# sota-zk-labs/zkp-implementation

Measured on AMD Instinct MI355X. Metric: G1 MSM scalar-muls/sec, higher is better.
Workload: dtype u32 (unsaturated 28-bit-limb Montgomery, 381-bit Fq; 64-bit accumulate)

## Files before the change

zkp-implementation_amd/csrc/msm.hpp:

```cpp
#pragma once
#include "g1.hpp"
#include "g1_28.hpp"
#include "fq28_inv.hpp"
#include "msm_plan.hpp"
#include "glv.hpp"

namespace zkp {

#define ZKP_AT(f, o) offsetof(MsmGeom, f) == o
static_assert(sizeof(MsmGeom) == 160 && ZKP_AT(c, 0) && ZKP_AT(nwin, 4) && ZKP_AT(nb, 8) && ZKP_AT(nchunk, 12) && ZKP_AT(n, 16) && ZKP_AT(chunk, 24) &&
              ZKP_AT(ns, 32) && ZKP_AT(plane_stride, 40) && ZKP_AT(nslice, 48) && ZKP_AT(shared, 52) && ZKP_AT(run_limit, 56) && ZKP_AT(piece, 60) &&
              ZKP_AT(resume, 64) && ZKP_AT(off, 68) && ZKP_AT(interleave, 140) && ZKP_AT(split_log, 144) && ZKP_AT(more, 148) && ZKP_AT(glv, 152), "MsmGeom layout");
#undef ZKP_AT
static_assert(sizeof(SortGeom) == 8 && offsetof(SortGeom, lo_bits) == 0 && offsetof(SortGeom, nhi) == 4, "SortGeom layout");

ZKP_DEV uint64_t bucket_cap(const MsmGeom& g) { return (uint64_t)g.nwin * g.nb; }

#ifdef ZKP_MSM_CHECK
__device__ uint32_t g_msm_check[32];
ZKP_DEV bool msm_check_fail(int cls, uint32_t v0, uint32_t v1) {
    if (atomicAdd(&g_msm_check[cls * 4], 1u) == 0) { g_msm_check[cls * 4 + 1] = v0; g_msm_check[cls * 4 + 2] = v1; }
    return true;
}
#endif
struct DigitSources {
    const Fr* scalars[MSM_MAX_BATCH];
};
ZKP_DEV void msm_recode(const uint32_t (&k)[8], bool skip, const MsmGeom& g, uint32_t nwin1, uint32_t group, uint64_t i,
                        uint32_t* __restrict__ digits) {
    const uint32_t win_off = group * nwin1;
    uint32_t carry = 0;
    for (uint32_t w = 0; w < nwin1; w++) {
        const uint32_t lo = g.off[w], width = (uint32_t)g.off[w + 1] - lo;
        const uint32_t limb = lo >> 5, sh = lo & 31;
        uint64_t v = 0;
#pragma unroll
        for (int q = 0; q < 8; q++) {
            if (q == (int)limb) v |= (uint64_t)k[q];
            if (q == (int)limb + 1) v |= (uint64_t)k[q] << 32;
        }
        uint32_t u = ((uint32_t)(v >> sh) & ((1u << width) - 1)) + carry;
        uint32_t enc;
        if (u > (1u << (width - 1))) {
            enc = (((1u << width) - u) << 1) | 1u;
            carry = 1;
        } else {
            enc = u << 1;
            carry = 0;
        }
        digits[(uint64_t)(win_off + w) * g.ns + i] = skip ? 0u : enc;
    }
}
__global__ __launch_bounds__(MSM_THREADS) void msm_digits_kernel(DigitSources src, const uint8_t* __restrict__ base_inf, MsmGeom g,
                                                                uint32_t nwin1, uint32_t* __restrict__ digits) {
    const uint64_t i = (uint64_t)blockIdx.x * MSM_THREADS + threadIdx.x;
    if (i >= g.ns) return;
    Fr k = from_mont(src.scalars[blockIdx.y][i]);
    const bool skip = base_inf != nullptr && base_inf[i] != 0;
    msm_recode(k.l, skip, g, nwin1, blockIdx.y, i, digits);
}
__global__ __launch_bounds__(MSM_THREADS) void msm_digits_glv_kernel(DigitSources src, const uint8_t* __restrict__ base_inf, MsmGeom g,
                                                                    uint32_t nwin1, uint32_t* __restrict__ digits) {
    const uint64_t i = (uint64_t)blockIdx.x * MSM_THREADS + threadIdx.x;
    if (i >= g.ns) return;
    const Fr k = from_mont(src.scalars[blockIdx.y][i]);
    const bool skip = base_inf != nullptr && base_inf[i] != 0;
    const GlvHalves h = glv_split(k.l);
    const uint32_t k1[8] = {h.k1[0], h.k1[1], h.k1[2], h.k1[3], 0, 0, 0, 0}, k2[8] = {h.k2[0], h.k2[1], h.k2[2], h.k2[3], 0, 0, 0, 0};
    msm_recode(k1, skip, g, nwin1, 2 * blockIdx.y, i, digits);
    msm_recode(k2, skip, g, nwin1, 2 * blockIdx.y + 1, i, digits);
}


ZKP_DEV void wave_exclusive_scan(const uint32_t* cnt, uint32_t* base, uint32_t nbins, uint32_t lane) {
    const uint32_t per = (nbins + 63) / 64;
    const uint32_t b0 = lane * per < nbins ? lane * per : nbins;
    const uint32_t b1 = b0 + per < nbins ? b0 + per : nbins;
    uint32_t sum = 0;
    for (uint32_t k = b0; k < b1; k++) sum += cnt[k];
    uint32_t inc = sum;
#pragma unroll
    for (int off = 1; off < 64; off <<= 1) {
        const uint32_t t = __shfl_up(inc, off);
        if (lane >= (uint32_t)off) inc += t;
    }
    uint32_t run = inc - sum;
    for (uint32_t k = b0; k < b1; k++) {
        const uint32_t v = cnt[k];
        base[k] = run;
        run += v;
    }
    if (lane == 63) base[nbins] = run;
}

__global__ __launch_bounds__(1024) void msm_parthist_kernel(const uint32_t* __restrict__ digits, MsmGeom g, SortGeom sg,
                                                            uint32_t* __restrict__ cntA) {
    __shared__ uint32_t h[SORT_MAX_PART];
    const uint32_t q = blockIdx.x, w = blockIdx.y;
    for (uint32_t k = threadIdx.x; k < sg.nhi; k += blockDim.x) h[k] = 0;
    __syncthreads();
    const uint64_t begin = (uint64_t)q * g.chunk;
    const uint64_t end = begin + g.chunk < g.n ? begin + g.chunk : g.n;
    const uint32_t* d = digits + (uint64_t)w * g.n;
    const uint64_t nt = blockDim.x;
    for (uint64_t i = begin + threadIdx.x; i < end; i += 4 * nt) {
        uint32_t e[4];
#pragma unroll
        for (int k = 0; k < 4; k++) e[k] = i + k * nt < end ? d[i + k * nt] : 0u;
#pragma unroll
        for (int k = 0; k < 4; k++) {
            const uint32_t b = e[k] >> 1;
            if (b) atomicAdd(&h[(b - 1) >> sg.lo_bits], 1u);
        }
    }
    __syncthreads();
    uint32_t* out = cntA + ((uint64_t)w * g.nchunk + q) * sg.nhi;
    for (uint32_t k = threadIdx.x; k < sg.nhi; k += blockDim.x) out[k] = h[k];
}

__global__ __launch_bounds__(1024) void msm_partprefix_kernel(uint32_t* __restrict__ cntA, MsmGeom g, SortGeom sg,
                                                              uint32_t* __restrict__ tot) {
    __shared__ uint32_t part[16][64];
    const uint32_t w = blockIdx.y, h = threadIdx.x & 63, qg = threadIdx.x >> 6;
    const uint32_t hi = blockIdx.x * 64 + h;
    const bool live = hi < sg.nhi;
    uint32_t* cw = cntA + (uint64_t)w * g.nchunk * sg.nhi;
    const uint32_t per = (g.nchunk + 15) / 16;
    const uint32_t q0 = qg * per < g.nchunk ? qg * per : g.nchunk;
    const uint32_t q1 = q0 + per < g.nchunk ? q0 + per : g.nchunk;
    uint32_t sum = 0;
    if (live)
        for (uint32_t q = q0; q < q1; q++) sum += cw[(uint64_t)q * sg.nhi + hi];
    part[qg][h] = sum;
    __syncthreads();
    uint32_t run = 0, total = 0;
    for (uint32_t k = 0; k < 16; k++) {
        if (k < qg) run += part[k][h];
        total += part[k][h];
    }
    if (live) {
        for (uint32_t q = q0; q < q1; q++) {
            uint32_t* p = cw + (uint64_t)q * sg.nhi + hi;
            const uint32_t v = *p;
            *p = run;
            run += v;
        }
        if (qg == 0) tot[(uint64_t)w * sg.nhi + hi] = total;
    }
}

__global__ __launch_bounds__(64) void msm_partstart_kernel(const uint32_t* __restrict__ tot, SortGeom sg,
                                                           uint32_t* __restrict__ pstart, uint32_t* __restrict__ ghist,
                                                           uint32_t* __restrict__ tail_barrier) {
    __shared__ uint32_t t[SORT_MAX_PART + 1];
    uint32_t* base = t;
    const uint32_t w = blockIdx.x;
    for (uint32_t k = threadIdx.x; k < 256; k += 64) {
        ghist[w * 256 + k] = 0;
        ghist[(gridDim.x + w) * 256 + k] = 0;
    }
    if (threadIdx.x == 0) tail_barrier[w * PYR_BAR_STRIDE] = 0;
    for (uint32_t k = threadIdx.x; k < sg.nhi; k += 64) t[k] = tot[(uint64_t)w * sg.nhi + k];
    __syncthreads();
    wave_exclusive_scan(t, base, sg.nhi, threadIdx.x);
    __syncthreads();
    for (uint32_t k = threadIdx.x; k <= sg.nhi; k += 64) pstart[(uint64_t)w * (sg.nhi + 1) + k] = base[k];
}

#ifndef ZKP_BS_TILE
#define ZKP_BS_TILE 16384
#endif
constexpr int BS_TILE = ZKP_BS_TILE;
constexpr int BS_PER = BS_TILE / 1024;
constexpr int SORT_MAX_BINS = 1024;

template <int PS_TILE>
__global__ __launch_bounds__(1024) void msm_partscatter_kernel(const uint32_t* __restrict__ digits, MsmGeom g, SortGeom sg,
                                                               const uint32_t* __restrict__ cntA,
                                                               const uint32_t* __restrict__ pstart,
                                                               uint2* __restrict__ entries) {
    constexpr int PS_PER = PS_TILE / 1024;
    extern __shared__ uint4 zkp_smem[];
    uint2* stage = reinterpret_cast<uint2*>(zkp_smem);
    uint16_t* part = reinterpret_cast<uint16_t*>(stage + PS_TILE);
    uint32_t* cur = reinterpret_cast<uint32_t*>(part + PS_TILE);
    uint32_t* cnt = cur + sg.nhi;
    uint32_t* base = cnt + sg.nhi;
    const uint32_t q = blockIdx.x, w = blockIdx.y, tid = threadIdx.x;
    for (uint32_t k = tid; k < sg.nhi; k += 1024)
        cur[k] = pstart[(uint64_t)w * (sg.nhi + 1) + k] + cntA[((uint64_t)w * g.nchunk + q) * sg.nhi + k];
    const uint64_t begin = (uint64_t)q * g.chunk;
    const uint64_t end = begin + g.chunk < g.n ? begin + g.chunk : g.n;
    const uint32_t* d = digits + (uint64_t)w * g.n;
    uint2* out = entries + (uint64_t)w * g.n;
    const uint32_t lo_mask = (1u << sg.lo_bits) - 1;
    for (uint64_t t0 = begin; t0 < end; t0 += PS_TILE) {
        for (uint32_t k = tid; k < sg.nhi; k += 1024) cnt[k] = 0;
        __syncthreads();
        uint32_t e[PS_PER], rk[PS_PER];
#pragma unroll
        for (int k = 0; k < PS_PER; k++) {
            const uint64_t i = t0 + tid + (uint64_t)k * 1024;
            e[k] = i < end ? d[i] : 0u;
        }
#pragma unroll
        for (int k = 0; k < PS_PER; k++) {
            const uint32_t b = e[k] >> 1;
            rk[k] = b ? atomicAdd(&cnt[(b - 1) >> sg.lo_bits], 1u) : 0u;
        }
        __syncthreads();
        if (tid < 64) wave_exclusive_scan(cnt, base, sg.nhi, tid);
        __syncthreads();
#pragma unroll
        for (int k = 0; k < PS_PER; k++) {
            const uint32_t b = e[k] >> 1;
            if (b) {
                const uint32_t p = (b - 1) >> sg.lo_bits;
                const uint32_t pos = base[p] + rk[k];
                stage[pos] = make_uint2((uint32_t)(t0 - 0 + tid + (uint64_t)k * 1024) | ((e[k] & 1u) << 31), (b - 1) & lo_mask);
// ... 39 lines not shown
        for (int k = 0; k < 4; k++)
            if (y[k] != 0xffffffffu) atomicAdd(&cnt[y[k]], 1u);
    }
    __syncthreads();
    if (tid < lo_n) atomicAdd(&szh[255 - (cnt[tid] < 255 ? cnt[tid] : 255)], 1u);
    if (tid < 64) wave_exclusive_scan(cnt, h, lo_n, tid);
    __syncthreads();
    if (tid < 256 && szh[tid]) atomicAdd(&ghist[w * 256 + tid], szh[tid]);
    if (tid < lo_n) h[tid] += begin;
    __syncthreads();
    uint32_t* sw = start + (uint64_t)w * (g.nb + 2);
    if (tid < lo_n) sw[(hi << sg.lo_bits) + tid + 1] = h[tid];
    if (hi == 0 && tid == 0) sw[0] = 0;
    if (hi == sg.nhi - 1 && tid == 0) sw[g.nb + 1] = end;
    __syncthreads();
    uint32_t* out = sorted + (uint64_t)w * g.n;
    for (uint32_t t0 = begin; t0 < end; t0 += BS_TILE) {
        if (tid < lo_n) cnt[tid] = 0;
        __syncthreads();
        uint2 e[BS_PER];
        uint32_t rk[BS_PER];
#pragma unroll
        for (int k = 0; k < BS_PER; k++) {
            const uint32_t i = t0 + tid + k * 1024;
            e[k] = i < end ? in[i] : make_uint2(0u, 0xffffffffu);
        }
#pragma unroll
        for (int k = 0; k < BS_PER; k++) rk[k] = e[k].y != 0xffffffffu ? atomicAdd(&cnt[e[k].y], 1u) : 0u;
        __syncthreads();
        if (tid < 64) wave_exclusive_scan(cnt, base, lo_n, tid);
        __syncthreads();
#pragma unroll
        for (int k = 0; k < BS_PER; k++)
            if (e[k].y != 0xffffffffu) {
                const uint32_t pos = base[e[k].y] + rk[k];
                stage[pos] = e[k].x;
                bin[pos] = (uint16_t)e[k].y;
            }
        __syncthreads();
        const uint32_t total = base[lo_n];
        for (uint32_t j = tid; j < total; j += 1024) {
            const uint32_t p = bin[j];
#ifdef ZKP_MSM_CHECK
            if ((uint64_t)h[p] + (j - base[p]) >= g.n && msm_check_fail(1, h[p] + (j - base[p]), p)) continue;
#endif
            out[h[p] + (j - base[p])] = stage[j];
        }
        __syncthreads();
        if (tid < lo_n) h[tid] += cnt[tid];
    }
}


__global__ __launch_bounds__(1024) void msm_rank_kernel(const uint32_t* __restrict__ start, MsmGeom g,
                                                        const uint32_t* __restrict__ ghist, uint32_t* __restrict__ gcur,
                                                        uint32_t* __restrict__ perm) {
    __shared__ uint32_t hist[256], base[256], gh[256], first[257];
    const uint32_t w = blockIdx.y, tid = threadIdx.x;
    const uint32_t* sw = start + (uint64_t)w * (g.nb + 2);
    if (tid < 256) {
        hist[tid] = 0;
        gh[tid] = ghist[w * 256 + tid];
    }
    __syncthreads();
    if (tid < 64) wave_exclusive_scan(gh, first, 256, tid);
    const uint32_t b = 1 + blockIdx.x * 1024 + tid;
    uint32_t bin = 0, rk = 0;
    if (b <= g.nb) {
        const uint32_t sz = sw[b + 1] - sw[b];
        bin = 255 - (sz < 255 ? sz : 255);
        rk = atomicAdd(&hist[bin], 1u);
    }
    __syncthreads();
    if (tid < 256 && hist[tid]) base[tid] = first[tid] + atomicAdd(&gcur[w * 256 + tid], hist[tid]);
    __syncthreads();
#ifdef ZKP_MSM_CHECK
    if (b <= g.nb && base[bin] + rk >= g.nb && msm_check_fail(5, base[bin] + rk, b)) return;
#endif
    if (b <= g.nb) perm[(uint64_t)w * g.nb + base[bin] + rk] = b;
}

__global__ __launch_bounds__(1024) void msm_order_kernel(const uint32_t* __restrict__ start, MsmGeom g,
                                                         const uint32_t* __restrict__ ghist,
                                                         const uint32_t* __restrict__ perm, uint32_t* __restrict__ over,
                                                         uint32_t* __restrict__ over_b, uint32_t* __restrict__ over_off,
                                                         uint4* __restrict__ desc, uint32_t over_cap, uint32_t desc_cap) {
    __shared__ uint32_t s_over[2], gh[256], first[257];
    const uint32_t w = blockIdx.x, tid = threadIdx.x, nt = blockDim.x;
    const uint32_t* sw = start + (uint64_t)w * (g.nb + 2);
    const uint32_t* pw = perm + (uint64_t)w * g.nb;
    if (tid < 256) gh[tid] = ghist[w * 256 + tid];
    __syncthreads();
    if (tid < 64) wave_exclusive_scan(gh, first, 256, tid);
    __syncthreads();
    if (tid == 0) {
        const uint32_t limit_bin = g.run_limit < 254 ? g.run_limit : 254;
        s_over[0] = first[255 - limit_bin];
    }
    __syncthreads();
    const uint32_t n_over = s_over[0] < over_cap ? s_over[0] : over_cap;
#ifdef ZKP_MSM_CHECK
    if (tid == 0 && s_over[0] > g.nb) msm_check_fail(7, s_over[0], over_cap);
#endif
    uint32_t* ob = over_b + (uint64_t)w * over_cap;
    uint32_t* oo = over_off + (uint64_t)w * (over_cap + 1);
    {
        __shared__ uint32_t part[1024];
        const uint32_t per = (n_over + nt - 1) / nt;
        const uint32_t r0 = tid * per < n_over ? tid * per : n_over;
        const uint32_t r1 = r0 + per < n_over ? r0 + per : n_over;
        uint32_t local = 0;
        for (uint32_t r = r0; r < r1; r++) {
            const uint32_t b = pw[r];
#ifdef ZKP_MSM_CHECK
            if ((b == 0 || b > g.nb) && msm_check_fail(6, b, r)) continue;
#endif
            const uint32_t sz = sw[b + 1] - sw[b];
            local += sz > g.run_limit ? (sz + g.piece - 1) / g.piece : 0;
        }
        part[tid] = local;
        __syncthreads();
        for (uint32_t off = 1; off < nt; off <<= 1) {
            const uint32_t v = tid >= off ? part[tid - off] : 0;
            __syncthreads();
            part[tid] += v;
            __syncthreads();
        }
        uint32_t run = tid ? part[tid - 1] : 0;
        for (uint32_t r = r0; r < r1; r++) {
            const uint32_t b = pw[r];
#ifdef ZKP_MSM_CHECK
            if (b == 0 || b > g.nb) { ob[r] = 1; oo[r] = run; continue; }
#endif
            const uint32_t sz = sw[b + 1] - sw[b];
            ob[r] = b;
            oo[r] = run;
            run += sz > g.run_limit ? (sz + g.piece - 1) / g.piece : 0;
        }
        if (tid == nt - 1) {
            const uint32_t total = part[nt - 1];
            oo[n_over] = total;
            s_over[1] = total;
            over[2 * w] = n_over;
            over[2 * w + 1] = total < desc_cap ? total : desc_cap;
        }
    }
    __syncthreads();
    const uint32_t n_pieces = s_over[1] < desc_cap ? s_over[1] : desc_cap;
    uint4* dw = desc + (uint64_t)w * desc_cap;
    for (uint32_t j = tid; j < n_pieces; j += nt) {
        uint32_t lo = 0, hi = n_over;
        while (hi - lo > 1) {
            const uint32_t mid = (lo + hi) >> 1;
            if (oo[mid] <= j) lo = mid; else hi = mid;
        }
        const uint32_t b = ob[lo], p = j - oo[lo];
        const uint32_t first = sw[b] + p * g.piece;
        const uint32_t last = first + g.piece < sw[b + 1] ? first + g.piece : sw[b + 1];
        dw[j] = make_uint4(b, p, first, last);
    }
}

__global__ __launch_bounds__(MSM_THREADS) void g1_to_internal_kernel(const uint4* __restrict__ in, uint64_t n,
                                                                    uint4* __restrict__ out) {
    const uint64_t i = (uint64_t)blockIdx.x * MSM_THREADS + threadIdx.x;
    if (i >= n) return;
    G1Affine p = G1Affine::load(in + i * 6);
#pragma unroll 1
    for (int k = 0; k < 8; k++) {
        p.x = dbl(p.x);
        p.y = dbl(p.y);
    }
    A28 q;
    q.x = fq28_from_sat(p.x);
    q.y = fq28_from_sat(p.y);
    q.store(out + i * 8);
}

struct SliceOffsets {
    uint16_t off[36];
};
__global__ __launch_bounds__(MSM_THREADS) void g1_expand_planes_kernel(uint4* __restrict__ planes, uint4* __restrict__ scratch,
                                                                      uint64_t off, uint64_t cnt, uint64_t plane_stride,
                                                                      uint32_t nplanes, SliceOffsets so) {
    const uint64_t j = (uint64_t)blockIdx.x * MSM_THREADS + threadIdx.x;
    if (j >= cnt) return;
    const uint64_t i = off + j;
    auto slot = [&](uint32_t s, uint32_t t) { return scratch + (((uint64_t)s * 3 + t) * cnt + j) * 4; };
    const A28 p0 = A28::load(planes + i * 8);
    X28 x = g1_28_double_affine(p0);
    Fq28 run = Fq28::one();
#pragma unroll 1
    for (uint32_t s = 1; s < nplanes; s++) {
#pragma unroll 1
        for (uint32_t k = (s == 1 ? 1u : 0u), c = (uint32_t)so.off[s] - so.off[s - 1]; k < c; k++) x = g1_28_double(x);
        A28 raw;
        raw.x = x.x;
        raw.y = x.y;
        raw.store(planes + (s * plane_stride + i) * 8);
        run.store(slot(s, 2));
        x.zz.store(slot(s, 0));
        x.zzz.store(slot(s, 1));
        run = run * x.zzz;
    }
    Fq28 inv = fq28_inverse_gcd(run);
#pragma unroll 1
    for (uint32_t s = nplanes - 1; s >= 1; s--) {
        const Fq28 zi3 = inv * Fq28::load(slot(s, 2));
        inv = inv * Fq28::load(slot(s, 1));
        const Fq28 zi = zi3 * Fq28::load(slot(s, 0));
        const Fq28 zi2 = zi * zi;
        uint4* dst = planes + (s * plane_stride + i) * 8;
        const A28 raw = A28::load(dst);
// ... 491 lines not shown
```

zkp-implementation_amd/csrc/msm_host.inc:

```

#ifdef ZKP_MSM_CHECK
#define MSM_TRACE(stream, ridx, what) do { hipError_t e_ = hipStreamSynchronize(stream); fprintf(stderr, "ZKP_MSM_CHECK range %llu: %s done (%d)\n", (unsigned long long)(ridx), what, (int)e_); } while (0)
#else
#define MSM_TRACE(stream, ridx, what) do { } while (0)
#endif

struct MsmFeed {
    const uint64_t* h_scalars;
    hipStream_t copy_stream;
    hipEvent_t ev;
    MsmFeedRanges ranges;
};

struct RangeBuffers {
    uint32_t *sorted, *start, *perm;
    uint4* desc;
    uint32_t *over, *over_b, *over_off;
};

struct MsmPass {
    const MsmPlan& p;
    const zkp_bases* bases;
    const Fr* const* scalars;
    size_t count;
// ... 65 lines not shown
                      });
        }
        hipError_t e1 = hipMemcpyAsync(dst, feed->h_scalars, 32 * p.lens[0], hipMemcpyHostToDevice, feed->copy_stream);
        if (e1 == hipSuccess) e1 = hipEventRecord(feed->ev, feed->copy_stream);
        up.release(e1 == hipSuccess);
        HIPCHK(e1);
        return ZKP_OK;
    }

    int walk() {
        if (p.overlap) {
            ZCHK(cx.sort_stream.ensure(hipStreamNonBlocking));
            for (Event* e : {&cx.ev_sort[0], &cx.ev_sort[1], &cx.ev_acc[0], &cx.ev_acc[1], &cx.ev_begin}) ZCHK(e->ensure(hipEventDisableTiming));
            sst = cx.sort_stream;
            HIPCHK(hipEventRecord(cx.ev_begin, st));
            HIPCHK(hipStreamWaitEvent(sst, cx.ev_begin, 0));
        }
        for (size_t ridx = 0; ridx < p.lens.size(); ridx++) {
            const MsmRange r = range_geom(p, ridx);
            const size_t par = r.set;
            const RangeBuffers rb = range_buffers(par);
            if (p.overlap && ridx >= 2) HIPCHK(hipStreamWaitEvent(sst, cx.ev_acc[par], 0));
            if (feed) {
                if (ridx == 0)
                    ZCHK(feed_first_range());
                else if (!up.wait_issued(ridx))
                    return fail(ZKP_E_DEVICE, "upload of a scalar range failed");
                HIPCHK(hipStreamWaitEvent(sst, ridx == 0 ? feed->ev : cx.copy_events[ridx - 1], 0));
            }
            launch_sort(rb, r);
            if (p.overlap) {
                HIPCHK(hipEventRecord(cx.ev_sort[par], sst));
                HIPCHK(hipStreamWaitEvent(st, cx.ev_sort[par], 0));
            }
            launch_accumulate(rb, r);
            if (p.overlap) HIPCHK(hipEventRecord(cx.ev_acc[par], st));
        }
        return ZKP_OK;
    }

    template <int TILE> void launch_partscatter(const MsmGeom& g) {
        hipLaunchKernelGGL(msm_partscatter_kernel<TILE>, dim3(g.nchunk, g.nwin), dim3(1024), p.ps_lds, sst,
                           cx.digits.get(), g, p.sg, cx.counts.get(), pstart, cx.entries.get());
    }
    void launch_sort(const RangeBuffers& rb, const MsmRange& r) {
        const SortGeom& sg = p.sg;
        const MsmGeom& g = r.g;
        const SortLaunch sl = sort_launch(sg, g);
        {
            ProfScope ps("msm_digits", sst);
            DigitSources ds;
            for (size_t m = 0; m < count; m++) ds.scalars[m] = scalars[m] + r.off;
            hipLaunchKernelGGL(g.glv ? msm_digits_glv_kernel : msm_digits_kernel, dim3(sl.digits_x, (unsigned)count), dim3(MSM_THREADS), 0,
                               sst, ds, bases->d_inf.p ? bases->d_inf.get() + r.off : nullptr, g, p.nwin1, cx.digits.get());
            MSM_TRACE(sst, r.ridx, "digits");
        }
        ProfScope ps("msm_sort", sst, true);
        hipLaunchKernelGGL(msm_parthist_kernel, dim3(g.nchunk, g.nwin), dim3(1024), 0, sst, cx.digits.get(), g, sg, cx.counts.get());
        MSM_TRACE(sst, r.ridx, "parthist");
        hipLaunchKernelGGL(msm_partprefix_kernel, dim3(sl.prefix_x, g.nwin), dim3(1024), 0, sst, cx.counts.get(), g, sg, ptot);
        hipLaunchKernelGGL(msm_partstart_kernel, dim3(g.nwin), dim3(64), 0, sst, ptot, sg, pstart, ghist, cx.result.get());
        MSM_TRACE(sst, r.ridx, "partprefix + partstart");
        switch (p.ps_tile) {
            case PS_TILE_SMALL: launch_partscatter<PS_TILE_SMALL>(g); break;
            case PS_TILE_MID: launch_partscatter<PS_TILE_MID>(g); break;
            default: launch_partscatter<PS_TILE_BIG>(g); break;
        }
        MSM_TRACE(sst, r.ridx, "partscatter");
        hipLaunchKernelGGL(msm_binsort_kernel, dim3(sg.nhi, g.nwin), dim3(1024), 0, sst, cx.entries.get(), g, sg, pstart, rb.start, rb.sorted, ghist);
        MSM_TRACE(sst, r.ridx, "binsort");
        hipLaunchKernelGGL(msm_rank_kernel, dim3(sl.rank_x, g.nwin), dim3(1024), 0, sst, rb.start, g, ghist, gcur, rb.perm);
        MSM_TRACE(sst, r.ridx, "rank");
        hipLaunchKernelGGL(msm_order_kernel, dim3(g.nwin), dim3(1024), 0, sst, rb.start, g, ghist, rb.perm, rb.over, rb.over_b, rb.over_off,
                           rb.desc, p.over_cap, p.desc_cap);
        MSM_TRACE(sst, r.ridx, "order");
    }

    void launch_accumulate(const RangeBuffers& rb, const MsmRange& r) {
        ProfScope ps("msm_accumulate", st, true);
        const MsmGeom& g = r.g;
        const AccLaunch a = acc_launch(p, g);
        const uint4* xy = static_cast<const uint4*>(bases->d_xy.p) + r.off * 8;
        uint4 *buckets = cx.buckets.get(), *pieces = cx.pieces.get(), *parts = cx.parts.get(), *carry = cx.pyr1.get();
        if (a.quad)
            hipLaunchKernelGGL(msm_accumulate_quad_kernel, dim3(a.grid), dim3(ACC_THREADS), 0, st, xy, rb.sorted, rb.start, rb.perm, rb.over, rb.desc,
                               p.desc_cap, a.bucket_blocks, a.extra_blocks, g, buckets, pieces, parts, clk_record(CLK_MSM_ACCUMULATE));
        else
            hipLaunchKernelGGL(msm_accumulate_kernel, dim3(a.grid), dim3(ACC_THREADS), 0, st, xy, rb.sorted, rb.start, rb.perm, rb.over, rb.desc,
                               p.desc_cap, a.bucket_blocks, a.extra_blocks, g, buckets, pieces, parts, carry, clk_record(CLK_MSM_ACCUMULATE));
        MSM_TRACE(st, r.ridx, "accumulate");
        hipLaunchKernelGGL(msm_combine_kernel, dim3(a.combine_x, g.nwin), dim3(64), 0, st, rb.over, rb.over_b,
                           rb.over_off, p.over_cap, p.desc_cap, g, pieces, buckets, carry);
        MSM_TRACE(st, r.ridx, "combine");
        for (uint32_t t = 0; t < g.split_log; t++)
            hipLaunchKernelGGL(p.fold[t].lane ? msm_fold_parts_lane_kernel : msm_fold_parts_kernel, dim3(p.fold[t].grid_x, p.fold[t].pairs),
                               dim3(MSM_THREADS), 0, st, buckets, parts, (uint64_t)g.nwin * g.nb, t);
    }

    void reduce() {
        const MsmGeom& g = p.g;
        const ReducePlan& red = p.red;
        for (size_t w = 0; w < W; w++) __atomic_store_n(result_flags + w, MSM_FLAG_PENDING, __ATOMIC_RELEASE);
        uint4* pyr[2] = {cx.buckets.get(), cx.pyr1.get()};
        uint4* odd[2] = {cx.odd0.get(), cx.odd1.get()};
        ProfScope ps("msm_bucket_reduce", st, true);
        for (uint32_t k = 0; k < red.nlevel; k++) {
            const PyrLaunch& v = red.level[k];
            const uint32_t l = v.level;
            hipLaunchKernelGGL(v.quad ? msm_pyramid_quad_kernel : msm_pyramid_kernel, dim3(v.grid_x, l + 1, g.nwin), dim3(MSM_THREADS), 0, st,
                               pyr[l & 1], pyr[(l + 1) & 1], odd[l & 1], odd[(l + 1) & 1], PyrLevel{l, v.half, g.nb, g.nwin});
        }
        if (red.tail_blocks) {
            const bool starve = knob_flag(KNOB_TEST_TAIL_STARVE);
            hipLaunchKernelGGL(msm_pyramid_tail_kernel, dim3(red.tail_blocks, g.nwin), dim3(red.tail_threads), 0, st, pyr[0], pyr[1], odd[0], odd[1],
                               red.nlevel, g.c, g.nb, cx.result.get(), result_out, result_flags, red.tail_blocks + (starve ? 1 : 0),
                               starve ? (1u << 12) : PYR_TAIL_SPIN_LIMIT);
        } else {
            const uint32_t fin = (g.c - 1) & 1;
            hipLaunchKernelGGL(msm_collect_kernel, dim3(g.nwin), dim3(64), 0, st, pyr[fin], pyr[fin ^ 1], odd[fin], g.nb, g.c, result_out,
                               result_flags);
        }
    }
};

int wait_msm_result(bool poll, size_t nwin, const uint32_t* flags, hipStream_t st) {
    ZCHK(poll_or_sync(poll && !knob_flag(KNOB_MSM_NO_POLL), st, [&] {
        for (size_t w = 0; w < nwin; w++)
            if (__atomic_load_n(flags + w, __ATOMIC_ACQUIRE) & MSM_FLAG_PENDING) return false;
// ... 78 lines not shown
```

zkp-implementation_amd/csrc/msm_plan.hpp:

```cpp
#pragma once
#include <algorithm>
#include <cstddef>
#include <cstdint>
#include <cstdlib>
#include <vector>

#include "../../include/zkp_hip.h"
#include "knobs.hpp"

namespace zkp {

#ifdef ZKP_HD
#define ZKP_MSMPLAN_FN ZKP_HD
#else
#define ZKP_MSMPLAN_FN inline
#endif

struct MsmGeom {
    uint32_t c;
    uint32_t nwin;
    uint32_t nb;
    uint32_t nchunk;
    uint64_t n;
    uint64_t chunk;
// ... 153 lines not shown
        const uint32_t per = quad ? MSM_THREADS / 4 : MSM_THREADS;
        r->level[l] = {l, half, quad ? 1u : 0u, (half + per - 1) / per};
    }
    r->nlevel = level_tail;
    r->tail_threads = tail_threads;
    r->tail_blocks = 0;
    if (level_tail + 1 < c) {
        uint32_t tb = tail_blocks;
        while (tb > 1 && (uint64_t)tb * nwin * (tail_threads / 64) > tail_max_waves) tb >>= 1;
        r->tail_blocks = tb;
    }
    return ZKP_OK;
}

struct FoldStep { uint32_t pairs, lane, grid_x; };

struct MsmPlan {
    MsmGeom g;
    SortGeom sg;
    std::vector<uint64_t> lens;
    uint64_t range;
    bool overlap;
    uint32_t nwin1, over_cap, desc_cap;
    size_t nbuf, over_bytes;
    MsmSizes bytes;
    FoldStep fold[MSM_MAX_SPLIT_LOG];
    ReducePlan red;
    bool poll_result;
    int ps_tile;
    size_t ps_lds;
    const char* error;
};

ZKP_MSMPLAN_FN bool acc_quad(const MsmGeom& g) { return !g.resume && !g.more && (uint64_t)g.n * g.nwin <= (1ull << 20); }

struct MsmRange {
    uint64_t off, len;
    uint32_t ridx, set;
    MsmGeom g;
};
inline MsmRange range_geom(const MsmPlan& p, size_t ridx) {
    MsmRange r{0, p.lens[ridx], (uint32_t)ridx, p.overlap ? (uint32_t)(ridx & 1) : 0u, p.g};
    for (size_t k = 0; k < ridx; k++) r.off += p.lens[k];
    if (r.len != p.g.ns) {
        r.g.ns = r.len;
        r.g.n = (uint64_t)p.nwin1 * r.len;
        r.g.chunk = (r.g.n + r.g.nchunk - 1) / r.g.nchunk;
    }
    r.g.resume = r.off ? 1u : 0u;
    r.g.more = ridx + 1 < p.lens.size() ? 1u : 0u;
    return r;
}

struct SortLaunch { uint32_t digits_x, prefix_x, rank_x; };
inline SortLaunch sort_launch(const SortGeom& sg, const MsmGeom& g) {
    return {(uint32_t)((g.ns + MSM_THREADS - 1) / MSM_THREADS), (sg.nhi + 63) / 64, (g.nb + 1023) / 1024};
}

struct AccLaunch { uint32_t quad, per_block, bucket_blocks, extra_blocks, grid, combine_x; };
inline AccLaunch acc_launch(const MsmPlan& p, const MsmGeom& g) {
    AccLaunch a;
    a.quad = acc_quad(g) ? 1u : 0u;
    a.per_block = a.quad ? ACC_THREADS / 4 : ACC_THREADS;
    a.bucket_blocks = (uint32_t)((((uint64_t)g.nb << g.split_log) + a.per_block - 1) / a.per_block);
    a.extra_blocks = std::min<uint32_t>((p.desc_cap + a.per_block - 1) / a.per_block, 64);
    a.grid = (a.bucket_blocks + a.extra_blocks) * g.nwin;
    a.combine_x = std::min<uint32_t>(p.over_cap, 64);
    return a;
}

inline int plan_msm(const MsmBases& bases, size_t count, size_t n, const MsmFeedRanges* feed, uint32_t tail_max_waves, MsmPlan* p) {
    auto refuse = [p](int code, const char* msg) { p->error = msg; return code; };
    p->lens.clear();
    if (n > bases.n) return refuse(ZKP_E_SIZE, "more scalars than bases (kzg/src/scheme.rs:86)");
    if (count == 0 || n == 0) return ZKP_OK;
    if (n >= (1ull << 31)) return refuse(ZKP_E_ARG, "n >= 2^31");
    if (count > (size_t)MSM_MAX_BATCH) return refuse(ZKP_E_ARG, "batch of more than 64 MSMs");
    const bool shared = bases.pre_c != 0;
    const bool glv = shared && bases.glv != 0;
    const uint32_t sets = glv ? 2 : 1;
    if (sets * count > (size_t)MSM_MAX_BATCH)
        return refuse(ZKP_E_ARG, "batch of more than 32 MSMs over endomorphism-split bases (two bucket sets per MSM, 64 per pass)");
    MsmGeom& g = p->g = MsmGeom{};
    g.c = shared ? bases.pre_c : pick_window_bits(n);
    const uint32_t nwin1 = shared ? bases.pre_planes : 256 / g.c + (256 % g.c ? 1 : 0);
    p->nwin1 = g.nslice = nwin1;
    static_assert(sizeof(MsmGeom::off) / sizeof(uint16_t) == 36, "MsmGeom::off");
    if (nwin1 + 1 > 36) return refuse(ZKP_E_ARG, "more than 35 windows per scalar");
    for (uint32_t s = 0; s <= nwin1; s++) g.off[s] = shared ? bases.pre_off[s] : (uint16_t)(s * g.c);
    g.shared = shared ? 1u : 0u;
    g.glv = glv ? 1u : 0u;
    std::vector<uint64_t>& lens = p->lens;
    if (shared) {
        const uint64_t max_range = sets * bases.pre_planes <= 12 ? 1ull << 24 : 1ull << 23;
        uint64_t cap = feed ? std::min<uint64_t>(max_range, 1ull << feed->range_log) : max_range;
        if (const long long v = knob_int(KNOB_MSM_RANGE_LOG)) cap = 1ull << v;
        uint64_t want_first = feed ? feed->first_len : 0;
        if (!feed && count == 1) {
            const long long v = knob_int(KNOB_MSM_FIRST_PCT);
            if (v) want_first = std::max<uint64_t>(1024, ((uint64_t)n * v / 100) & ~(uint64_t)1023);
        }
        uint64_t done = 0;
        for (uint64_t want : {want_first, feed && want_first ? feed->second_len : (uint64_t)0})
            if (want && done + want < n) {
                lens.push_back(std::min<uint64_t>(want, cap));
                done += lens.back();
            }
        const uint64_t rest = n - done, rpass = (rest + cap - 1) / cap, rr = (rest + rpass - 1) / rpass;
        for (; done < n; done += lens.back()) lens.push_back(std::min<uint64_t>(rr, n - done));
// ... 52 lines not shown
```

Measured before the change: 448.4 million.

## Fuse sort-stage kernels with last-arriving-block tickets and stage recode limbs in LDS

Merges the partstart kernel into partprefix and the order kernel into rank. A per-window atomic ticket lets the last-arriving block perform the follow-on serial step, which removes two kernel launches and their dependency gaps. The ticket words are reset inside the digits kernel. Partprefix now uses smaller blocks and register-batched column loads, and digit recoding reads limbs from shared memory instead of a predicated select loop. The cost is extra cross-block synchronisation complexity and possible memory-ordering bugs.

```diff
diff --git a/zkp-implementation_amd/csrc/msm.hpp b/zkp-implementation_amd/csrc/msm.hpp
--- a/zkp-implementation_amd/csrc/msm.hpp
+++ b/zkp-implementation_amd/csrc/msm.hpp
@@ -26,20 +26,24 @@
 struct DigitSources {
     const Fr* scalars[MSM_MAX_BATCH];
 };
+constexpr int MSM_MAX_SLICES = 35;
+struct DigitLimbs {
+    uint32_t l[9][MSM_THREADS];
+};
 ZKP_DEV void msm_recode(const uint32_t (&k)[8], bool skip, const MsmGeom& g, uint32_t nwin1, uint32_t group, uint64_t i,
-                        uint32_t* __restrict__ digits) {
-    const uint32_t win_off = group * nwin1;
+                        uint32_t* __restrict__ digits, DigitLimbs& limbs) {
+    const uint32_t tid = threadIdx.x;
+#pragma unroll
+    for (int q = 0; q < 8; q++) limbs.l[q][tid] = skip ? 0u : k[q];
+    uint32_t* out = digits + (uint64_t)group * nwin1 * g.ns + i;
     uint32_t carry = 0;
-    for (uint32_t w = 0; w < nwin1; w++) {
+#pragma unroll
+    for (uint32_t w = 0; w < (uint32_t)MSM_MAX_SLICES; w++) {
+        if (w >= nwin1) continue;
         const uint32_t lo = g.off[w], width = (uint32_t)g.off[w + 1] - lo;
         const uint32_t limb = lo >> 5, sh = lo & 31;
-        uint64_t v = 0;
-#pragma unroll
-        for (int q = 0; q < 8; q++) {
-            if (q == (int)limb) v |= (uint64_t)k[q];
-            if (q == (int)limb + 1) v |= (uint64_t)k[q] << 32;
-        }
-        uint32_t u = ((uint32_t)(v >> sh) & ((1u << width) - 1)) + carry;
+        const uint64_t v = (uint64_t)limbs.l[limb][tid] | (uint64_t)limbs.l[limb + 1][tid] << 32;
+        const uint32_t u = ((uint32_t)(v >> sh) & ((1u << width) - 1)) + carry;
         uint32_t enc;
         if (u > (1u << (width - 1))) {
             enc = (((1u << width) - u) << 1) | 1u;
@@ -48,27 +52,39 @@
             enc = u << 1;
             carry = 0;
         }
-        digits[(uint64_t)(win_off + w) * g.ns + i] = skip ? 0u : enc;
-    }
+        out[(uint64_t)w * g.ns] = enc;
+    }
+}
+ZKP_DEV void msm_digits_prologue(const MsmGeom& g, uint32_t* __restrict__ bar, DigitLimbs& limbs) {
+    if (blockIdx.x == 0 && blockIdx.y == 0)
+        for (uint32_t w = threadIdx.x; w < g.nwin; w += MSM_THREADS) {
+            __hip_atomic_store(bar + (uint64_t)w * PYR_BAR_STRIDE + BAR_WORD_PREFIX, 0u, __ATOMIC_RELAXED, __HIP_MEMORY_SCOPE_AGENT);
+            __hip_atomic_store(bar + (uint64_t)w * PYR_BAR_STRIDE + BAR_WORD_RANK, 0u, __ATOMIC_RELAXED, __HIP_MEMORY_SCOPE_AGENT);
+        }
+    limbs.l[8][threadIdx.x] = 0;
 }
 __global__ __launch_bounds__(MSM_THREADS) void msm_digits_kernel(DigitSources src, const uint8_t* __restrict__ base_inf, MsmGeom g,
-                                                                uint32_t nwin1, uint32_t* __restrict__ digits) {
+                                                                uint32_t nwin1, uint32_t* __restrict__ digits, uint32_t* __restrict__ bar) {
+    __shared__ DigitLimbs limbs;
+    msm_digits_prologue(g, bar, limbs);
     const uint64_t i = (uint64_t)blockIdx.x * MSM_THREADS + threadIdx.x;
     if (i >= g.ns) return;
     Fr k = from_mont(src.scalars[blockIdx.y][i]);
     const bool skip = base_inf != nullptr && base_inf[i] != 0;
-    msm_recode(k.l, skip, g, nwin1, blockIdx.y, i, digits);
+    msm_recode(k.l, skip, g, nwin1, blockIdx.y, i, digits, limbs);
 }
 __global__ __launch_bounds__(MSM_THREADS) void msm_digits_glv_kernel(DigitSources src, const uint8_t* __restrict__ base_inf, MsmGeom g,
-                                                                    uint32_t nwin1, uint32_t* __restrict__ digits) {
+                                                                    uint32_t nwin1, uint32_t* __restrict__ digits, uint32_t* __restrict__ bar) {
+    __shared__ DigitLimbs limbs;
+    msm_digits_prologue(g, bar, limbs);
     const uint64_t i = (uint64_t)blockIdx.x * MSM_THREADS + threadIdx.x;
     if (i >= g.ns) return;
     const Fr k = from_mont(src.scalars[blockIdx.y][i]);
     const bool skip = base_inf != nullptr && base_inf[i] != 0;
     const GlvHalves h = glv_split(k.l);
     const uint32_t k1[8] = {h.k1[0], h.k1[1], h.k1[2], h.k1[3], 0, 0, 0, 0}, k2[8] = {h.k2[0], h.k2[1], h.k2[2], h.k2[3], 0, 0, 0, 0};
-    msm_recode(k1, skip, g, nwin1, 2 * blockIdx.y, i, digits);
-    msm_recode(k2, skip, g, nwin1, 2 * blockIdx.y + 1, i, digits);
+    msm_recode(k1, skip, g, nwin1, 2 * blockIdx.y, i, digits, limbs);
+    msm_recode(k2, skip, g, nwin1, 2 * blockIdx.y + 1, i, digits, limbs);
 }
 
 
@@ -118,53 +134,78 @@
     for (uint32_t k = threadIdx.x; k < sg.nhi; k += blockDim.x) out[k] = h[k];
 }
 
-__global__ __launch_bounds__(1024) void msm_partprefix_kernel(uint32_t* __restrict__ cntA, MsmGeom g, SortGeom sg,
-                                                              uint32_t* __restrict__ tot) {
-    __shared__ uint32_t part[16][64];
-    const uint32_t w = blockIdx.y, h = threadIdx.x & 63, qg = threadIdx.x >> 6;
-    const uint32_t hi = blockIdx.x * 64 + h;
+ZKP_DEV void handoff_store(uint32_t* p, uint32_t v) { __hip_atomic_store(p, v, __ATOMIC_RELAXED, __HIP_MEMORY_SCOPE_AGENT); }
+ZKP_DEV bool sort_last_arrival(uint32_t* ticket, uint32_t expect, uint32_t* s_last) {
+    asm volatile("s_waitcnt vmcnt(0)" ::: "memory");
+    __syncthreads();
+    if (expect == 1) return true;
+    if (threadIdx.x == 0) {
+        const bool last = __hip_atomic_fetch_add(ticket, 1u, __ATOMIC_RELAXED, __HIP_MEMORY_SCOPE_AGENT) + 1 == expect;
+        if (last) {
+            __builtin_amdgcn_fence(__ATOMIC_ACQUIRE, "agent");
+            asm volatile("s_waitcnt vmcnt(0)" ::: "memory");
+        }
+        *s_last = last ? 1u : 0u;
+    }
+    __syncthreads();
+    return *s_last != 0;
+}
+
+__global__ __launch_bounds__(PREFIX_THREADS) void msm_partprefix_kernel(uint32_t* __restrict__ cntA, MsmGeom g, SortGeom sg, uint32_t* tot,
+                                                                       uint32_t* __restrict__ pstart, uint32_t* __restrict__ ghist,
+                                                                       uint32_t* __restrict__ bar) {
+    __shared__ uint32_t part[PREFIX_GROUPS][PREFIX_COLS];
+    __shared__ uint32_t s_last;
+    __shared__ uint32_t t[SORT_MAX_PART + 1];
+    const uint32_t w = blockIdx.y, h = threadIdx.x % PREFIX_COLS, qg = threadIdx.x / PREFIX_COLS;
+    const uint32_t hi = blockIdx.x * PREFIX_COLS + h;
     const bool live = hi < sg.nhi;
     uint32_t* cw = cntA + (uint64_t)w * g.nchunk * sg.nhi;
-    const uint32_t per = (g.nchunk + 15) / 16;
+    const uint32_t per = (g.nchunk + PREFIX_GROUPS - 1) / PREFIX_GROUPS;
     const uint32_t q0 = qg * per < g.nchunk ? qg * per : g.nchunk;
     const uint32_t q1 = q0 + per < g.nchunk ? q0 + per : g.nchunk;
+    constexpr uint32_t PREFIX_KEEP = 32;
+    const bool keep = per <= PREFIX_KEEP;
+    const uint32_t qe = live ? q1 : q0;
+    uint32_t v[PREFIX_KEEP];
     uint32_t sum = 0;
-    if (live)
-        for (uint32_t q = q0; q < q1; q++) sum += cw[(uint64_t)q * sg.nhi + hi];
+    for (uint32_t qb = q0; qb < qe; qb += PREFIX_KEEP) {
+#pragma unroll
+        for (uint32_t k = 0; k < PREFIX_KEEP; k++) v[k] = qb + k < qe ? cw[(uint64_t)(qb + k) * sg.nhi + hi] : 0u;
+#pragma unroll
+        for (uint32_t k = 0; k < PREFIX_KEEP; k++) sum += v[k];
+    }
     part[qg][h] = sum;
     __syncthreads();
     uint32_t run = 0, total = 0;
-    for (uint32_t k = 0; k < 16; k++) {
+    for (uint32_t k = 0; k < PREFIX_GROUPS; k++) {
         if (k < qg) run += part[k][h];
         total += part[k][h];
     }
-    if (live) {
-        for (uint32_t q = q0; q < q1; q++) {
-            uint32_t* p = cw + (uint64_t)q * sg.nhi + hi;
-            const uint32_t v = *p;
-            *p = run;
-            run += v;
-        }
-        if (qg == 0) tot[(uint64_t)w * sg.nhi + hi] = total;
-    }
-}
-
-__global__ __launch_bounds__(64) void msm_partstart_kernel(const uint32_t* __restrict__ tot, SortGeom sg,
-                                                           uint32_t* __restrict__ pstart, uint32_t* __restrict__ ghist,
-                                                           uint32_t* __restrict__ tail_barrier) {
-    __shared__ uint32_t t[SORT_MAX_PART + 1];
-    uint32_t* base = t;
-    const uint32_t w = blockIdx.x;
-    for (uint32_t k = threadIdx.x; k < 256; k += 64) {
+    for (uint32_t qb = q0; qb < qe; qb += PREFIX_KEEP) {
+        if (!keep) {
+#pragma unroll
+            for (uint32_t k = 0; k < PREFIX_KEEP; k++) v[k] = qb + k < qe ? cw[(uint64_t)(qb + k) * sg.nhi + hi] : 0u;
+        }
+#pragma unroll
+        for (uint32_t k = 0; k < PREFIX_KEEP; k++)
+            if (qb + k < qe) {
+                cw[(uint64_t)(qb + k) * sg.nhi + hi] = run;
+                run += v[k];
+            }
+    }
+    if (live && qg == 0) handoff_store(tot + (uint64_t)w * sg.nhi + hi, total);
+    if (!sort_last_arrival(bar + (uint64_t)w * PYR_BAR_STRIDE + BAR_WORD_PREFIX, gridDim.x, &s_last)) return;
+    for (uint32_t k = threadIdx.x; k < 256; k += PREFIX_THREADS) {
         ghist[w * 256 + k] = 0;
-        ghist[(gridDim.x + w) * 256 + k] = 0;
-    }
-    if (threadIdx.x == 0) tail_barrier[w * PYR_BAR_STRIDE] = 0;
-    for (uint32_t k = threadIdx.x; k < sg.nhi; k += 64) t[k] = tot[(uint64_t)w * sg.nhi + k];
-    __syncthreads();
-    wave_exclusive_scan(t, base, sg.nhi, threadIdx.x);
-    __syncthreads();
-    for (uint32_t k = threadIdx.x; k <= sg.nhi; k += 64) pstart[(uint64_t)w * (sg.nhi + 1) + k] = base[k];
+        ghist[(gridDim.y + w) * 256 + k] = 0;
+    }
+    if (threadIdx.x == 0) __hip_atomic_store(bar + (uint64_t)w * PYR_BAR_STRIDE + BAR_WORD_TAIL, 0u, __ATOMIC_RELAXED, __HIP_MEMORY_SCOPE_AGENT);
+    for (uint32_t k = threadIdx.x; k < sg.nhi; k += PREFIX_THREADS) t[k] = tot[(uint64_t)w * sg.nhi + k];
+    __syncthreads();
+    if (threadIdx.x < 64) wave_exclusive_scan(t, t, sg.nhi, threadIdx.x);
+    __syncthreads();
+    for (uint32_t k = threadIdx.x; k <= sg.nhi; k += PREFIX_THREADS) pstart[(uint64_t)w * (sg.nhi + 1) + k] = t[k];
 }
 
 #ifndef ZKP_BS_TILE
@@ -310,55 +351,19 @@
 }
 
 
-__global__ __launch_bounds__(1024) void msm_rank_kernel(const uint32_t* __restrict__ start, MsmGeom g,
-                                                        const uint32_t* __restrict__ ghist, uint32_t* __restrict__ gcur,
-                                                        uint32_t* __restrict__ perm) {
-    __shared__ uint32_t hist[256], base[256], gh[256], first[257];
-    const uint32_t w = blockIdx.y, tid = threadIdx.x;
-    const uint32_t* sw = start + (uint64_t)w * (g.nb + 2);
-    if (tid < 256) {
-        hist[tid] = 0;
-        gh[tid] = ghist[w * 256 + tid];
-    }
-    __syncthreads();
-    if (tid < 64) wave_exclusive_scan(gh, first, 256, tid);
-    const uint32_t b = 1 + blockIdx.x * 1024 + tid;
-    uint32_t bin = 0, rk = 0;
-    if (b <= g.nb) {
-        const uint32_t sz = sw[b + 1] - sw[b];
-        bin = 255 - (sz < 255 ? sz : 255);
-        rk = atomicAdd(&hist[bin], 1u);
-    }
-    __syncthreads();
-    if (tid < 256 && hist[tid]) base[tid] = first[tid] + atomicAdd(&gcur[w * 256 + tid], hist[tid]);
-    __syncthreads();
+
+ZKP_DEV uint32_t msm_order_candidates(const uint32_t* first, const MsmGeom& g) {
+    const uint32_t limit_bin = g.run_limit < 254 ? g.run_limit : 254;
+    return first[255 - limit_bin];
+}
+ZKP_DEV void msm_order_body(uint32_t w, const uint32_t* __restrict__ sw, const uint32_t* pw, uint32_t n_cand, const MsmGeom& g,
+                            uint32_t* __restrict__ over, uint32_t* __restrict__ over_b, uint32_t* __restrict__ over_off,
+                            uint4* __restrict__ desc, uint32_t over_cap, uint32_t desc_cap) {
+    __shared__ uint32_t s_over[2];
+    const uint32_t tid = threadIdx.x, nt = blockDim.x;
+    const uint32_t n_over = n_cand < over_cap ? n_cand : over_cap;
 #ifdef ZKP_MSM_CHECK
-    if (b <= g.nb && base[bin] + rk >= g.nb && msm_check_fail(5, base[bin] + rk, b)) return;
-#endif
-    if (b <= g.nb) perm[(uint64_t)w * g.nb + base[bin] + rk] = b;
-}
-
-__global__ __launch_bounds__(1024) void msm_order_kernel(const uint32_t* __restrict__ start, MsmGeom g,
-                                                         const uint32_t* __restrict__ ghist,
-                                                         const uint32_t* __restrict__ perm, uint32_t* __restrict__ over,
-                                                         uint32_t* __restrict__ over_b, uint32_t* __restrict__ over_off,
-                                                         uint4* __restrict__ desc, uint32_t over_cap, uint32_t desc_cap) {
-    __shared__ uint32_t s_over[2], gh[256], first[257];
-    const uint32_t w = blockIdx.x, tid = threadIdx.x, nt = blockDim.x;
-    const uint32_t* sw = start + (uint64_t)w * (g.nb + 2);
-    const uint32_t* pw = perm + (uint64_t)w * g.nb;
-    if (tid < 256) gh[tid] = ghist[w * 256 + tid];
-    __syncthreads();
-    if (tid < 64) wave_exclusive_scan(gh, first, 256, tid);
-    __syncthreads();
-    if (tid == 0) {
-        const uint32_t limit_bin = g.run_limit < 254 ? g.run_limit : 254;
-        s_over[0] = first[255 - limit_bin];
-    }
-    __syncthreads();
-    const uint32_t n_over = s_over[0] < over_cap ? s_over[0] : over_cap;
-#ifdef ZKP_MSM_CHECK
-    if (tid == 0 && s_over[0] > g.nb) msm_check_fail(7, s_over[0], over_cap);
+    if (tid == 0 && n_cand > g.nb) msm_check_fail(7, n_cand, over_cap);
 #endif
     uint32_t* ob = over_b + (uint64_t)w * over_cap;
     uint32_t* oo = over_off + (uint64_t)w * (over_cap + 1);
@@ -413,10 +418,52 @@
             if (oo[mid] <= j) lo = mid; else hi = mid;
         }
         const uint32_t b = ob[lo], p = j - oo[lo];
-        const uint32_t first = sw[b] + p * g.piece;
-        const uint32_t last = first + g.piece < sw[b + 1] ? first + g.piece : sw[b + 1];
-        dw[j] = make_uint4(b, p, first, last);
-    }
+        const uint32_t first_e = sw[b] + p * g.piece;
+        const uint32_t last_e = first_e + g.piece < sw[b + 1] ? first_e + g.piece : sw[b + 1];
+        dw[j] = make_uint4(b, p, first_e, last_e);
+    }
+}
+
+__global__ __launch_bounds__(1024) void msm_rank_kernel(const uint32_t* __restrict__ start, MsmGeom g,
+                                                        const uint32_t* __restrict__ ghist, uint32_t* __restrict__ gcur, uint32_t* perm,
+                                                        uint32_t* __restrict__ over, uint32_t* __restrict__ over_b,
+                                                        uint32_t* __restrict__ over_off, uint4* __restrict__ desc, uint32_t over_cap,
+                                                        uint32_t desc_cap, uint32_t* __restrict__ bar) {
+    __shared__ uint32_t hist[256], base[256], gh[256], first[257], s_last;
+    const uint32_t w = blockIdx.y, tid = threadIdx.x;
+    const uint32_t* sw = start + (uint64_t)w * (g.nb + 2);
+    if (tid < 256) {
+        hist[tid] = 0;
+        gh[tid] = ghist[w * 256 + tid];
+    }
+    __syncthreads();
+    if (tid < 64) wave_exclusive_scan(gh, first, 256, tid);
+    const uint32_t b = 1 + blockIdx.x * 1024 + tid;
+    uint32_t bin = 0, rk = 0;
+    if (b <= g.nb) {
+        const uint32_t sz = sw[b + 1] - sw[b];
+        bin = 255 - (sz < 255 ? sz : 255);
+        rk = atomicAdd(&hist[bin], 1u);
+    }
+    __syncthreads();
+    if (tid < 256 && hist[tid]) base[tid] = first[tid] + atomicAdd(&gcur[w * 256 + tid], hist[tid]);
+    __syncthreads();
+    bool put = b <= g.nb;
+#ifdef ZKP_MSM_CHECK
+    if (put && base[bin] + rk >= g.nb && msm_check_fail(5, base[bin] + rk, b)) put = false;
+#endif
+    const uint32_t n_cand = msm_order_candidates(first, g);
+    if (put) {
+        const uint32_t r = base[bin] + rk;
+        if (r < n_cand) handoff_store(perm + (uint64_t)w * g.nb + r, b);
+        else perm[(uint64_t)w * g.nb + r] = b;
+    }
+    if (n_cand == 0) {
+        if (blockIdx.x != 0) return;
+    } else if (!sort_last_arrival(bar + (uint64_t)w * PYR_BAR_STRIDE + BAR_WORD_RANK, gridDim.x, &s_last)) {
+        return;
+    }
+    msm_order_body(w, sw, perm + (uint64_t)w * g.nb, n_cand, g, over, over_b, over_off, desc, over_cap, desc_cap);
 }
 
 __global__ __launch_bounds__(MSM_THREADS) void g1_to_internal_kernel(const uint4* __restrict__ in, uint64_t n,
diff --git a/zkp-implementation_amd/csrc/msm_host.inc b/zkp-implementation_amd/csrc/msm_host.inc
--- a/zkp-implementation_amd/csrc/msm_host.inc
+++ b/zkp-implementation_amd/csrc/msm_host.inc
@@ -141,15 +141,15 @@
             DigitSources ds;
             for (size_t m = 0; m < count; m++) ds.scalars[m] = scalars[m] + r.off;
             hipLaunchKernelGGL(g.glv ? msm_digits_glv_kernel : msm_digits_kernel, dim3(sl.digits_x, (unsigned)count), dim3(MSM_THREADS), 0,
-                               sst, ds, bases->d_inf.p ? bases->d_inf.get() + r.off : nullptr, g, p.nwin1, cx.digits.get());
+                               sst, ds, bases->d_inf.p ? bases->d_inf.get() + r.off : nullptr, g, p.nwin1, cx.digits.get(), cx.result.get());
             MSM_TRACE(sst, r.ridx, "digits");
         }
         ProfScope ps("msm_sort", sst, true);
         hipLaunchKernelGGL(msm_parthist_kernel, dim3(g.nchunk, g.nwin), dim3(1024), 0, sst, cx.digits.get(), g, sg, cx.counts.get());
         MSM_TRACE(sst, r.ridx, "parthist");
-        hipLaunchKernelGGL(msm_partprefix_kernel, dim3(sl.prefix_x, g.nwin), dim3(1024), 0, sst, cx.counts.get(), g, sg, ptot);
-        hipLaunchKernelGGL(msm_partstart_kernel, dim3(g.nwin), dim3(64), 0, sst, ptot, sg, pstart, ghist, cx.result.get());
-        MSM_TRACE(sst, r.ridx, "partprefix + partstart");
+        hipLaunchKernelGGL(msm_partprefix_kernel, dim3(sl.prefix_x, g.nwin), dim3(PREFIX_THREADS), 0, sst, cx.counts.get(), g, sg, ptot, pstart,
+                           ghist, cx.result.get());
+        MSM_TRACE(sst, r.ridx, "partprefix");
         switch (p.ps_tile) {
             case PS_TILE_SMALL: launch_partscatter<PS_TILE_SMALL>(g); break;
             case PS_TILE_MID: launch_partscatter<PS_TILE_MID>(g); break;
@@ -158,11 +158,9 @@
         MSM_TRACE(sst, r.ridx, "partscatter");
         hipLaunchKernelGGL(msm_binsort_kernel, dim3(sg.nhi, g.nwin), dim3(1024), 0, sst, cx.entries.get(), g, sg, pstart, rb.start, rb.sorted, ghist);
         MSM_TRACE(sst, r.ridx, "binsort");
-        hipLaunchKernelGGL(msm_rank_kernel, dim3(sl.rank_x, g.nwin), dim3(1024), 0, sst, rb.start, g, ghist, gcur, rb.perm);
-        MSM_TRACE(sst, r.ridx, "rank");
-        hipLaunchKernelGGL(msm_order_kernel, dim3(g.nwin), dim3(1024), 0, sst, rb.start, g, ghist, rb.perm, rb.over, rb.over_b, rb.over_off,
-                           rb.desc, p.over_cap, p.desc_cap);
-        MSM_TRACE(sst, r.ridx, "order");
+        hipLaunchKernelGGL(msm_rank_kernel, dim3(sl.rank_x, g.nwin), dim3(1024), 0, sst, rb.start, g, ghist, gcur, rb.perm, rb.over, rb.over_b,
+                           rb.over_off, rb.desc, p.over_cap, p.desc_cap, cx.result.get());
+        MSM_TRACE(sst, r.ridx, "rank + order");
     }
 
     void launch_accumulate(const RangeBuffers& rb, const MsmRange& r) {
diff --git a/zkp-implementation_amd/csrc/msm_plan.hpp b/zkp-implementation_amd/csrc/msm_plan.hpp
--- a/zkp-implementation_amd/csrc/msm_plan.hpp
+++ b/zkp-implementation_amd/csrc/msm_plan.hpp
@@ -229,9 +229,13 @@
     return r;
 }
 
+constexpr uint32_t PREFIX_COLS = 16, PREFIX_GROUPS = 16, PREFIX_THREADS = PREFIX_COLS * PREFIX_GROUPS;
+constexpr uint32_t BAR_WORD_TAIL = 0, BAR_WORD_PREFIX = 1, BAR_WORD_RANK = 2;
+static_assert(BAR_WORD_RANK < PYR_BAR_STRIDE, "the tickets live in the free words of a window's barrier line");
+
 struct SortLaunch { uint32_t digits_x, prefix_x, rank_x; };
 inline SortLaunch sort_launch(const SortGeom& sg, const MsmGeom& g) {
-    return {(uint32_t)((g.ns + MSM_THREADS - 1) / MSM_THREADS), (sg.nhi + 63) / 64, (g.nb + 1023) / 1024};
+    return {(uint32_t)((g.ns + MSM_THREADS - 1) / MSM_THREADS), (sg.nhi + PREFIX_COLS - 1) / PREFIX_COLS, (g.nb + 1023) / 1024};
 }
 
 struct AccLaunch { uint32_t quad, per_block, bucket_blocks, extra_blocks, grid, combine_x; };
```

Measured after the change: 439.0 million. 0.979x the previous value.
